# liyangSKD/slam-eslam

Measured on AMD Instinct MI355X. Metric: M particle-updates/s (predict+weight+resample) @ 1/2/4/8 MI355X, higher is better.
Workload: dtype f64; 1 GPU; configs[2]: 4194304 particles/GPU, 1 MI355X per rank, MLS 1000x1000 @0.1 m, 4 contacts, resample forced every step; particles_per_gpu=4194304, global_particles=4194304, parallelism=dp1 (particle shards)

## Files before the change

include/eslam_detmath.h:

```cpp
#ifndef ESLAM_DETMATH_H
#define ESLAM_DETMATH_H

#include <stdint.h>

#if defined(__HIPCC__)
#define DM_FN __host__ __device__ static inline __attribute__((always_inline))
#define DM_CONST static constexpr
#define DM_UNROLL _Pragma("unroll")
#else
#define DM_FN static inline
#define DM_CONST static const
#define DM_UNROLL
#endif

DM_FN uint64_t dm_bits(double x) { uint64_t u; __builtin_memcpy(&u, &x, 8); return u; }
DM_FN double dm_from_bits(uint64_t u) { double x; __builtin_memcpy(&x, &u, 8); return x; }
DM_FN uint32_t dm_fbits(float x) { uint32_t u; __builtin_memcpy(&u, &x, 4); return u; }
DM_FN int dm_isnan(double x) { return x != x; }
DM_FN int dm_isfinite(double x) { return (dm_bits(x) & 0x7ff0000000000000ull) != 0x7ff0000000000000ull; }
DM_FN double dm_fabs(double x) { return dm_from_bits(dm_bits(x) & 0x7fffffffffffffffull); }
DM_FN double dm_fma(double a, double b, double c) { return __builtin_fma(a, b, c); }
#if defined(__HIP_DEVICE_COMPILE__)
DM_FN double dm_fmak(double a, double b, double k)
{
// ... 757 lines not shown
    {-0.47139673682599764, 0.881921264348355},
    {-0.4496113296546066, 0.8932243011955153},
    {-0.4275550934302821, 0.9039892931234433},
    {-0.40524131400498986, 0.9142097557035307},
    {-0.3826834323650898, 0.9238795325112867},
    {-0.35989503653498817, 0.9329927988347388},
    {-0.33688985339222005, 0.9415440651830208},
    {-0.31368174039889146, 0.9495281805930367},
    {-0.2902846772544624, 0.9569403357322088},
    {-0.26671275747489837, 0.9637760657954398},
    {-0.2429801799032639, 0.970031253194544},
    {-0.2191012401568698, 0.9757021300385286},
    {-0.19509032201612828, 0.9807852804032304},
    {-0.17096188876030122, 0.9852776423889412},
    {-0.14673047445536175, 0.989176509964781},
    {-0.1224106751992162, 0.99247953459871},
    {-0.0980171403295606, 0.9951847266721969},
    {-0.07356456359966743, 0.9972904566786902},
    {-0.049067674327418015, 0.9987954562051724},
    {-0.024541228522912288, 0.9996988186962042},
};
#define DM_BM_DELTA 1.4629180792671596e-09

DM_FN double dm_log_bm(double u)
{
    const uint64_t b = dm_bits(u);
    const uint32_t hi = (uint32_t)(b >> 32);
    const int32_t t = (int32_t)(hi - 0x3fe80000u);
    const int32_t k = t >> 20;
    const uint32_t i = ((uint32_t)t >> 13) & 127u;
    const double z = dm_from_bits(((uint64_t)(hi - ((uint32_t)t & 0xfff00000u)) << 32) | (b & 0xffffffffull));
    const double* e = dm_bm_log_tab[i];
    const double r = dm_fma(z, e[0], -1.0);
    double p = dm_fmak(r, 1.0 / 7.0, -1.0 / 6.0);
    p = dm_fmak(p, r, 0.2);
    p = dm_fmak(p, r, -0.25);
    p = dm_fmak(p, r, 1.0 / 3.0);
    p = dm_fma_mh(p, r);
    const double l1p = dm_fma(r * r, p, r);
    const double kd = (double)k;
    const double h = kd * DM_LN2_HI + e[1];
    const double l = kd * DM_LN2_LO + e[2];
    return h + (l1p + l);
}

DM_FN void dm_sincos2pi32(uint32_t b, double* s, double* c)
{
    const double* e = dm_bm_sc_tab[b >> 24];
    const double d = ((double)(b & 0xffffffu) + 0.5) * DM_BM_DELTA;
    const double z = d * d;
    double ps = dm_fmak(z, -1.0 / 5040.0, 1.0 / 120.0);
    ps = dm_fmak(ps, z, -1.0 / 6.0);
    const double sd = dm_fma(d * z, ps, d);
    double pc = dm_fmak(z, 1.0 / 40320.0, -1.0 / 720.0);
    pc = dm_fmak(pc, z, 1.0 / 24.0);
    pc = dm_fma_mh(pc, z);
    const double cd = dm_fma_1(pc, z);
    *s = dm_fma(e[0], cd, e[1] * sd);
    *c = dm_fma(e[1], cd, -(e[0] * sd));
}

DM_CONST float dm_bm_sc_tab32[256][2] = {
    {0.0f, 1.0f},
    {0.024541229009628296f, 0.99969881772995f},
    {0.049067676067352295f, 0.9987954497337341f},
    {0.0735645666718483f, 0.9972904324531555f},
// ... 234 lines not shown
    {-0.4275550842285156f, 0.903989315032959f},
    {-0.40524131059646606f, 0.91420978307724f},
    {-0.3826834261417389f, 0.9238795042037964f},
    {-0.3598950505256653f, 0.9329928159713745f},
    {-0.3368898630142212f, 0.9415440559387207f},
    {-0.3136817514896393f, 0.949528157711029f},
    {-0.290284663438797f, 0.9569403529167175f},
    {-0.2667127549648285f, 0.9637760519981384f},
    {-0.24298018217086792f, 0.9700312614440918f},
    {-0.21910123527050018f, 0.9757021069526672f},
    {-0.19509032368659973f, 0.9807852506637573f},
    {-0.1709618866443634f, 0.9852776527404785f},
    {-0.1467304676771164f, 0.9891765117645264f},
    {-0.12241067737340927f, 0.9924795627593994f},
    {-0.0980171412229538f, 0.9951847195625305f},
    {-0.0735645666718483f, 0.9972904324531555f},
    {-0.049067676067352295f, 0.9987954497337341f},
    {-0.024541229009628296f, 0.99969881772995f},
};
#define DM_BM_DELTA_F 1.462918119976564e-09f

DM_FN float dm_fmaf(float a, float b, float c) { return __builtin_fmaf(a, b, c); }

DM_FN void dm_sincos2pi32f(uint32_t b, float* s, float* c)
{
    const float* e = dm_bm_sc_tab32[b >> 24];
    const float d = dm_fmaf((float)(b & 0xffffffu), DM_BM_DELTA_F, 0.5f * DM_BM_DELTA_F);
    const float z = d * d;
    const float sd = dm_fmaf(d * z, -1.0f / 6.0f, d);
    const float cd = dm_fmaf(z, dm_fmaf(z, 1.0f / 24.0f, -0.5f), 1.0f);
    *s = dm_fmaf(e[0], cd, e[1] * sd);
    *c = dm_fmaf(e[1], cd, -(e[0] * sd));
}

DM_FN float dm_sqrtf_pos(float x)
{
#if defined(__HIP_DEVICE_COMPILE__)
    const float r = __builtin_amdgcn_sqrtf(x);
    const float dn = __uint_as_float(__float_as_uint(r) - 1u), up = __uint_as_float(__float_as_uint(r) + 1u);
    float q = r;
    if (__builtin_fmaf(-dn, r, x) <= 0.0f) q = dn;
    if (__builtin_fmaf(-up, r, x) > 0.0f) q = up;
    return q;
#else
    return __builtin_sqrtf(x);
#endif
}

DM_FN void dm_box_muller32(uint32_t a, uint32_t b, double* z0, double* z1)
{
    const float r = dm_sqrtf_pos((float)(-2.0 * dm_log_bm(dm_u32(a))));
    float s, c;
    dm_sincos2pi32f(b, &s, &c);
    *z0 = (double)r * (double)c;
    *z1 = (double)r * (double)s;
}

#define DM_STREAM_PROJECT 1u
#define DM_STREAM_INIT 2u
#define DM_STREAM_HASH 3u

DM_FN dm_philox_ctr dm_draw(uint64_t seed, uint32_t stream, uint64_t ev, uint64_t gidx, uint32_t call)
{
    dm_philox_ctr c;
    c.v[0] = (uint32_t)gidx;
    c.v[1] = (uint32_t)(gidx >> 32);
    c.v[2] = (uint32_t)ev;
    c.v[3] = (stream << 24) | ((call & 0xffu) << 16) | (uint32_t)((ev >> 32) & 0xffffu);
    return dm_philox4x32_10(c, (uint32_t)seed, (uint32_t)(seed >> 32) ^ 0x5EED5EEDu);
}

#define DM_MINSTD_A 48271u
#define DM_MINSTD_M 2147483647u

DM_FN uint32_t dm_mulmod31(uint32_t a, uint32_t b)
{
    uint64_t p = (uint64_t)a * b;
    uint64_t r = (p & DM_MINSTD_M) + (p >> 31);
// ... 578 lines not shown
```

slam-eslam_amd/csrc/eslam_internal.h:

```cpp
#pragma once
#include <stdint.h>
#include "../../include/eslam_gpu.h"
#include "../../include/eslam_detmath.h"

namespace eslam_dev {

constexpr int kBlock = 256;
constexpr int kWaves = kBlock / 64;
constexpr int kScanItems = 8;
constexpr int kScanTile = kBlock * kScanItems;
constexpr int kGatherTile = kScanTile;
constexpr int kRow = 64;
constexpr int kNShard = 16;
constexpr int kJumpBits = 11;
constexpr int kStatsLds = 2048;
#ifndef ESLAM_WINDOW_LDS
#define ESLAM_WINDOW_LDS 29696
#endif
constexpr int kWindowLds = ESLAM_WINDOW_LDS;
#ifndef ESLAM_K1_ATTR
#define ESLAM_K1_ATTR
#endif

#if defined(__HIPCC__)
__device__ __forceinline__ uint32_t jump_pow(const uint32_t* __restrict__ jt, uint64_t e)
{
    uint32_t a = jt[e & 2047u];
    uint32_t b = jt[2048u + ((e >> 11) & 2047u)];
    uint32_t c = jt[4096u + ((e >> 22) & 1023u)];
    return dm_mulmod31(dm_mulmod31(a, b), c);
}
#endif

struct alignas(128) Shard {
    uint64_t A[DM_NBUCKETS][4];
    uint64_t B[DM_NBUCKETS][4];
    uint64_t SW[4];
    uint64_t D, TP;
    uint64_t maxm;
    uint64_t flags;
    uint64_t err;
    uint64_t bbox[4];
// ... 414 lines not shown
```

slam-eslam_amd/csrc/eslam_kernels.hip:

```cpp
#include <hip/hip_runtime.h>
#include <type_traits>
#include <string.h>

#include "eslam_internal.h"
#include "eslam_launch.h"

namespace eslam_dev {

template <int O> __device__ __forceinline__ uint32_t xor_lane_u32(uint32_t v)
{
    static_assert(O == 1 || O == 2 || O == 4 || O == 8 || O == 16 || O == 32, "xor distance");
    if constexpr (O == 32) {
        const auto r = __builtin_amdgcn_permlane32_swap(v, v, false, false);
        return (threadIdx.x & 32u) ? r[0] : r[1];
    } else if constexpr (O == 16) {
        const auto r = __builtin_amdgcn_permlane16_swap(v, v, false, false);
        return (threadIdx.x & 16u) ? r[0] : r[1];
    } else if constexpr (O == 8) {
        const int t = __builtin_amdgcn_update_dpp(0, (int)v, 0x108, 0xf, 0x3, false);
        return (uint32_t)__builtin_amdgcn_update_dpp(t, (int)v, 0x118, 0xf, 0xc, false);
    } else if constexpr (O == 4) {
        const int t = __builtin_amdgcn_update_dpp(0, (int)v, 0x104, 0xf, 0x5, false);
        return (uint32_t)__builtin_amdgcn_update_dpp(t, (int)v, 0x114, 0xf, 0xa, false);
    } else if constexpr (O == 2) {
// ... 121 lines not shown
{
    su2 r;
    asm volatile("s_load_dwordx2 %0, %1, %2\n\ts_waitcnt lgkmcnt(0)" : "=&s"(r) : "s"(kseg()), "s"(off));
    return r;
}
__device__ __forceinline__ su4 kl4(uint32_t off)
{
    su4 r;
    asm volatile("s_load_dwordx4 %0, %1, %2\n\ts_waitcnt lgkmcnt(0)" : "=&s"(r) : "s"(kseg()), "s"(off));
    return r;
}
__device__ __forceinline__ su8 kl8(uint32_t off)
{
    su8 r;
    asm volatile("s_load_dwordx8 %0, %1, %2\n\ts_waitcnt lgkmcnt(0)" : "=&s"(r) : "s"(kseg()), "s"(off));
    return r;
}
__device__ __forceinline__ su16 kl16(uint32_t off)
{
    su16 r;
    asm volatile("s_load_dwordx16 %0, %1, %2\n\ts_waitcnt lgkmcnt(0)" : "=&s"(r) : "s"(kseg()), "s"(off));
    return r;
}
__device__ __forceinline__ void kl8_2(uint32_t off_a, uint32_t off_b, su8& a, su2& b)
{
    asm volatile("s_load_dwordx8 %0, %2, %3\n\ts_load_dwordx2 %1, %2, %4\n\ts_waitcnt lgkmcnt(0)"
                 : "=&s"(a), "=&s"(b) : "s"(kseg()), "s"(off_a), "s"(off_b));
}
template <class V> __device__ __forceinline__ uint64_t kq(const V& r, int k)
{
    return (uint64_t)r[2 * k] | ((uint64_t)r[2 * k + 1] << 32);
}
template <class V> __device__ __forceinline__ double kd(const V& r, int k) { return dm_from_bits(kq(r, k)); }
template <class T> using gmem = __attribute__((address_space(1))) T;
template <class T, class V> __device__ __forceinline__ gmem<T>* kp(const V& r, int k) { return (gmem<T>*)(uintptr_t)kq(r, k); }

struct StatePtrs {
    gmem<double> *x, *y, *th, *z, *zs, *w, *mprob;
    gmem<uint8_t>* flags;
};
__device__ __forceinline__ StatePtrs kstate(uint32_t off)
{
    const su16 r = kl16(off);
    return StatePtrs{kp<double>(r, 0), kp<double>(r, 1), kp<double>(r, 2), kp<double>(r, 3),
                     kp<double>(r, 4), kp<double>(r, 5), kp<double>(r, 6), kp<uint8_t>(r, 7)};
}

static_assert(offsetof(StepParams, mu) == 24 && offsetof(StepParams, L22) == 88 && offsetof(StepParams, z_delta) == 120 &&
                  offsetof(StepParams, me2) == 136 && offsetof(StepParams, use_shape) == 168,
              "K1 scalar-load blocks");
static_assert(offsetof(MapView, width) == 48 && offsetof(MapView, height) == 64, "map lookup header");
static_assert(offsetof(ContactC, pz) == 32 && offsetof(GatherView, record) == 32, "K1 scalar-load blocks");
static_assert(offsetof(LocalMaps, S) == 24 && offsetof(LocalMaps, hy) == 40 && offsetof(LocalMaps, mx) == 48 &&
                  offsetof(LocalMaps, my) == 56, "K1 reads the local maps' first 64 bytes");

struct alignas(16) WinCell {
    float mean0, stdev0;
    uint32_t begin, count;
};

__shared__ __attribute__((aligned(16))) int k1_win[8];

struct Window {
    int on;
    const WinCell* cells;
};

struct WinBounds {
    int on, m0, m1, n0, n1, cols;
// ... 101 lines not shown
    for (int i = 0; i < N; ++i) {
        if (dm[i] == 0xffffffffu) continue;
        if (pg[i] == kStoreTrail) {
            fnd[i] = store_patch(sid, dm[i], dn[i], lz[i], qv, mean[i], stdev[i]);
        } else if (pg[i] != DM_LM_NONE) {
            const float sd = __uint_as_float((uint32_t)(pf[i] >> 32));
            fnd[i] = dm_lm_holds(sd) && patch_gate(nullptr, 0, __uint_as_float((uint32_t)pf[i]), sd, lz[i], qv, mean[i], stdev[i]);
        }
    }
}

__device__ __forceinline__ uint32_t store_sid(uint32_t sid)
{
    const su16 h = kl16(KOFF(store));
    const uint64_t w3 = kq(h, 3), w5 = kq(h, 5);
    const uint32_t S = (uint32_t)w3, V = (uint32_t)(w5 >> 32);
    const uint32_t f = kp<const uint32_t>(h, 1)[(uint64_t)sid * S + (S - 4u * V - 2u)];
    return sid | (f == kLmShadow ? 0x80000000u : 0u);
}

template <bool DELTA = false, bool DEFER = false>
__device__ __forceinline__ bool get_patch(const Window& win, double px, double py, double pz, double qv, double& mean,
                                          double& stdev, uint32_t sid = 0, uint32_t* dm = nullptr, uint32_t* dn = nullptr,
                                          double* dlz = nullptr)
{
    if constexpr (DEFER) *dm = 0xffffffffu;
    const su16 h = kl16(KOFF(map));
    const uint32_t width = h[12], hcells = h[13], ident = h[14], has_height = h[15];
    double lx = px, ly = py, lz = pz;
    if (!ident) {
        const su16 a = kl16(KOFF(map.g2l));
        const su8 b = kl8(KOFF(map.g2l[8]));
        lx = ((kd(a, 0) * px + kd(a, 1) * py) + kd(a, 2) * pz) + kd(a, 3);
        ly = ((kd(a, 4) * px + kd(a, 5) * py) + kd(a, 6) * pz) + kd(a, 7);
        lz = ((kd(b, 0) * px + kd(b, 1) * py) + kd(b, 2) * pz) + kd(b, 3);
    }
    const double ux = (lx - kd(h, 4)) * kd(h, 2);
    const double uy = (ly - kd(h, 5)) * kd(h, 3);
    if constexpr (DELTA) {
        if (sid >> 31) {
            sid &= 0x7fffffffu;
            const double fm = floor(ux), fn = floor(uy);
            if ((fm >= 0.0) & (fm < (double)width) & (fn >= 0.0) & (fn < (double)hcells) &&
                store_patch(sid, (uint32_t)fm, (uint32_t)fn, lz, qv, mean, stdev))
                return true;
        }
    }
    int im, in;
    asm("v_cvt_i32_f64 %0, %1" : "=v"(im) : "v"(ux));
    asm("v_cvt_i32_f64 %0, %1" : "=v"(in) : "v"(uy));
// ... 151 lines not shown
    return w;
}

struct CMResult {
    uint32_t ncp;
    bool accepted;
    double weight, zdelta, zvar, posevar, s2;
};

__device__ __forceinline__ bool ratio_surely_significant(double z, double zvar, double corr)
{
    const double s2 = zvar * (corr * corr);
    if (z <= 0.0) return s2 < 1e16;
    return s2 < 1600.0 && z * z < 31.36 * s2;
}

#ifndef ESLAM_K1_LB
#define ESLAM_K1_LB 4
#endif
constexpr int kK1LookupBatch = ESLAM_K1_LB;

template <int MAXP, bool BATCH, bool DELTA = false, bool UNG = false>
__device__ __forceinline__ CMResult evaluate_pose(const Window& win, double co, double s, double r22, double x, double y,
                                                  double z, double meas_var, uint32_t sid)
{
    CMResult r;
    double cz[MAXP], cv[MAXP];
    bool ok[MAXP];
#pragma unroll
    for (int k = 0; k < MAXP; ++k) ok[k] = false;
    uint32_t ncp = 0;
    bool valid = false, group_valid = true;
    double contact_ratio = 0, pose_var_avg = 0, posevar = 0;
    double pzd = 0, pzv = 0;
    const double qv = meas_var;
    const su8 wp = kl8(KOFF(p.me2));
    const su4 wq = kl4(KOFF(p.use_shape));
    const double radius = kd(wp, 1), corr = kd(wp, 2);
    const uint32_t m = wq[1], eval_mask = wq[2], end_mask = wq[3];

    auto push = [&](uint32_t i, double zd, double zv) {
        if constexpr (BATCH) {
            cz[i] = zd; cv[i] = zv; ok[i] = true;
        } else {
#pragma unroll
            for (int k = 0; k < MAXP; ++k)
                if ((uint32_t)k == ncp) { cz[k] = zd; cv[k] = zv; }
        }
        ++ncp;
    };
    auto contact = [&](uint32_t i, bool found, double mean, double stdev, double wz) {
        const bool c_eval = (eval_mask >> i) & 1u, c_end = (end_mask >> i) & 1u;
        if (group_valid && c_eval) {
            if (found) {
                const double zdiff = wz - mean;
                const double pose_var = stdev * stdev;
                const double zvar = stdev * stdev + meas_var;
                if (!valid && c_end && ratio_surely_significant(zdiff, zvar, corr)) {
                    posevar += pose_var;
                    push(i, zdiff, zvar);
// ... 14 lines not shown
                    pzv += zvar * ratio;
                    contact_ratio += ratio;
                    pose_var_avg += pose_var * ratio;
                }
                valid = true;
            } else {
                group_valid = false;
            }
        }
        if (valid && c_end) {
            if (group_valid && contact_ratio > 1e-9) {
                const double inv = 1.0 / contact_ratio;
                pzd *= inv;
                pzv *= inv;
                posevar += pose_var_avg * inv;
                push(i, pzd, pzv);
            }
            group_valid = true;
            valid = false;
            pose_var_avg = 0;
            contact_ratio = 0;
        }
    };
    auto world = [&](uint32_t i, double& wx, double& wy, double& wz) {
        su8 c;
        su2 cpz;
        const uint32_t off = KOFF(p.c) + i * (uint32_t)sizeof(ContactC);
        kl8_2(off, off + (uint32_t)offsetof(ContactC, pz), c, cpz);
        const double px = kd(c, 0), py = kd(c, 1), zp = kd(c, 2), zz = kd(c, 3), pz = kd(cpz, 0);
        wx = ((co * px + (-s) * py) + zp) + x;
        wy = ((s * px + co * py) + zp) + y;
        wz = ((zz + r22 * pz) + z) - radius;
    };
    auto lookup = [&](double wx, double wy, double wz, double& mean, double& stdev) -> bool {
        return get_patch<DELTA>(win, wx, wy, wz, qv, mean, stdev, sid);
    };

    if constexpr (BATCH && UNG && kK1LookupBatch < MAXP) {
        bool alive = true;
#pragma unroll
        for (int g = 0; g < MAXP; g += kK1LookupBatch) {
            bool fnd[kK1LookupBatch];
            double mn[kK1LookupBatch], sd[kK1LookupBatch], wzs[kK1LookupBatch];
#pragma unroll
            for (int q = 0; q < kK1LookupBatch; ++q) {
                const int i = g + q;
                fnd[q] = false; mn[q] = 0.0; sd[q] = 0.0; wzs[q] = 0.0;
                if ((uint32_t)i < m) {
                    double wx, wy;
                    world((uint32_t)i, wx, wy, wzs[q]);
                    if ((eval_mask >> i) & 1u) fnd[q] = lookup(wx, wy, wzs[q], mn[q], sd[q]);
                }
            }
#pragma unroll
            for (int q = 0; q < kK1LookupBatch; ++q) {
                const int i = g + q;
                if ((uint32_t)i >= m) break;
                if (!((eval_mask >> i) & 1u)) continue;
                if (alive && fnd[q]) {
                    const double zdiff = wzs[q] - mn[q];
                    const double pose_var = sd[q] * sd[q];
                    const double zvar = sd[q] * sd[q] + meas_var;
                    double pzd_i = zdiff, pzv_i = zvar, pv_i = pose_var;
                    bool take = true;
                    if (!ratio_surely_significant(zdiff, zvar, corr)) {
                        const double ratio = dm_normal_pdf_cdf_ratio(zdiff, dm_sqrt(zvar) * corr);
                        take = ratio > 1e-9;
                        const double inv = 1.0 / ratio;
                        pzd_i = (zdiff * ratio) * inv;
                        pzv_i = (zvar * ratio) * inv;
                        pv_i = (pose_var * ratio) * inv;
                    }
                    if (take) {
                        posevar += pv_i;
                        push((uint32_t)i, pzd_i, pzv_i);
                    }
                }
                alive = alive && fnd[q];
            }
        }
    } else if constexpr (BATCH) {
        bool fnd[MAXP];
        double mn[MAXP], sd[MAXP], wzs[MAXP];
        if constexpr (DELTA) {
            if (!(sid >> 31)) {
                uint32_t dm[MAXP], dn[MAXP];
                double dlz[MAXP];
#pragma unroll
                for (int i = 0; i < MAXP; ++i) {
                    fnd[i] = false; mn[i] = 0.0; sd[i] = 0.0; wzs[i] = 0.0; dm[i] = 0xffffffffu; dn[i] = 0u; dlz[i] = 0.0;
                    if ((uint32_t)i < m) {
                        double wx, wy;
                        world((uint32_t)i, wx, wy, wzs[i]);
                        if ((eval_mask >> i) & 1u)
                            fnd[i] = get_patch<true, true>(win, wx, wy, wzs[i], qv, mn[i], sd[i], sid, &dm[i], &dn[i], &dlz[i]);
                    }
                }
                store_patches<MAXP>(sid, dm, dn, dlz, qv, fnd, mn, sd);
            } else {
#pragma unroll
                for (int i = 0; i < MAXP; ++i) {
                    fnd[i] = false; mn[i] = 0.0; sd[i] = 0.0; wzs[i] = 0.0;
                    if ((uint32_t)i < m) {
                        double wx, wy;
                        world((uint32_t)i, wx, wy, wzs[i]);
                        if ((eval_mask >> i) & 1u) fnd[i] = lookup(wx, wy, wzs[i], mn[i], sd[i]);
                    }
                }
            }
        } else {
#pragma unroll
            for (int i = 0; i < MAXP; ++i) {
                fnd[i] = false; mn[i] = 0.0; sd[i] = 0.0; wzs[i] = 0.0;
                if ((uint32_t)i < m) {
                    double wx, wy;
                    world((uint32_t)i, wx, wy, wzs[i]);
                    if ((eval_mask >> i) & 1u) fnd[i] = lookup(wx, wy, wzs[i], mn[i], sd[i]);
                }
            }
        }
        if constexpr (UNG) {
            bool alive = true;
#pragma unroll
            for (int i = 0; i < MAXP; ++i) {
                if ((uint32_t)i >= m) break;
                if (!((eval_mask >> i) & 1u)) continue;
                if (alive && fnd[i]) {
                    const double zdiff = wzs[i] - mn[i];
                    const double pose_var = sd[i] * sd[i];
                    const double zvar = sd[i] * sd[i] + meas_var;
                    double pzd_i = zdiff, pzv_i = zvar, pv_i = pose_var;
                    bool take = true;
                    if (!ratio_surely_significant(zdiff, zvar, corr)) {
                        const double ratio = dm_normal_pdf_cdf_ratio(zdiff, dm_sqrt(zvar) * corr);
                        take = ratio > 1e-9;
                        const double inv = 1.0 / ratio;
                        pzd_i = (zdiff * ratio) * inv;
                        pzv_i = (zvar * ratio) * inv;
                        pv_i = (pose_var * ratio) * inv;
                    }
                    if (take) {
                        posevar += pv_i;
                        push((uint32_t)i, pzd_i, pzv_i);
                    }
                }
                alive = alive && fnd[i];
            }
        } else {
#pragma unroll
            for (int i = 0; i < MAXP; ++i) {
                if ((uint32_t)i >= m) break;
                contact((uint32_t)i, fnd[i], mn[i], sd[i], wzs[i]);
            }
        }
    } else {
        for (uint32_t i = 0; i < m; ++i) {
            double wx, wy, wz, mean = 0.0, stdev = 0.0;
            world(i, wx, wy, wz);
            bool found = false;
            if (group_valid && ((eval_mask >> i) & 1u)) found = lookup(wx, wy, wz, mean, stdev);
            contact(i, found, mean, stdev, wz);
        }
    }
    r.ncp = ncp;
    r.posevar = posevar;
    r.accepted = (uint64_t)ncp >= kq(wp, 3);
    r.weight = r.zdelta = r.zvar = r.s2 = 0.0;
    if (r.accepted) {
        double d1 = 0, d2 = 0, inv_d2;
        auto sums = [&](auto recip) {
#pragma unroll
            for (int k = 0; k < MAXP; ++k) {
                if (BATCH ? ok[k] : (uint32_t)k < ncp) {
                    cv[k] = recip(cv[k]);
                    d1 += cz[k] * cv[k];
                    d2 += cv[k];
                }
            }
            inv_d2 = recip(d2);
        };
        if (meas_var >= 0x1p-400 && meas_var <= 0x1p300) sums([](double v) { return dm_div_inrange(1.0, v); });
        else sums([](double v) { return 1.0 / v; });
        const double delta = d1 * inv_d2;
        double s2 = 0.0;
#pragma unroll
        for (int k = 0; k < MAXP; ++k) {
            if (BATCH ? ok[k] : (uint32_t)k < ncp) {
                const double d = cz[k] - delta;
                s2 += (d * d) * cv[k];
            }
        }
        r.s2 = s2;
        const uint32_t use_shape = kl2(KOFF(p.use_shape))[0];
        const double pz = use_shape ? dm_exp(-0.5 * s2) : 1.0;
        r.weight = pz;
        r.zdelta = -delta;
        r.zvar = inv_d2;
    }
    return r;
}

__device__ __forceinline__ uint32_t decode_source(uint32_t v, uint32_t multi, const gmem<const Rec>* __restrict__ recs,
                                                  const gmem<const Rec>** rec)
{
    *rec = nullptr;
    if (multi) {
        if (v >= kMarkOwn && v < kMarkHigh) return v - kMarkOwn;
        *rec = recs + (v >= kMarkHigh ? v - kMarkHigh : v);
        return 0;
    }
    return v;
}

#define K1_ST(p, v) __builtin_nontemporal_store((v), (p))

#ifndef ESLAM_K1D_WPE
// ... 10 lines not shown
    const uint64_t nchunks = (n + csz - 1) / csz;
    Ctl* ctl = a.ctl;
    if (ctl->err & kFaultTimeout) return;
    const uint32_t gath = ctl->gather;
    const uint32_t cur = ctl->base ^ ctl->flip;
    if (WEIGHT && blockIdx.x == 0 && threadIdx.x == 0) ctl->k3_base = cur;
    const uint32_t st_off = __builtin_amdgcn_readfirstlane(cur ? KOFF(s[1]) : KOFF(s[0]));
    const uint32_t si_off = __builtin_amdgcn_readfirstlane(gath ? (ctl->base ? KOFF(s[1]) : KOFF(s[0])) : st_off);
    const int wexp = ctl->wexp;
    double spread = 0.0;
    bool do_spread = false;
    double tf = 0.0, rf = 0.0;
    if (PROJECT) {
        spread = dm_weighting_function(ctl->max_weight, 0.0, a.p.spread_threshold, 0.0);
        do_spread = spread > 0 && !a.p.hash_use;
        tf = a.p.spread_trans * spread;
        rf = a.p.spread_rot * spread;
    }

    extern __shared__ __attribute__((aligned(16))) unsigned char smem[];
    Window win;
    win.on = 0;
    if (WEIGHT) win = stage_window(a.map, a.p, ctl, 6.0 * tf, smem + kStatsLds);
    ESLAM_STAMP(g_stamps_k1, 1);

    double maxm = 0.0;
    uint32_t nDTP = 0, werr = 0, flag = 0;
    uint32_t touched = 0;
    float bb[4] = {-INFINITY, -INFINITY, -INFINITY, -INFINITY};
    uint64_t limb = 0;
    const int sa = DM_FX_SCALE - wexp, sb = DM_FX_SCALE - 2 * wexp;

    uint64_t chunk = (uint64_t)blockIdx.x * kWaves + wave;
    bool active = chunk < nchunks;
    if (a.sel.mode == 1u) {
        active = chunk >= a.sel.cdev[0] && chunk < a.sel.cdev[1];
    } else if (a.sel.mode == 2u) {
        chunk = chunk < a.sel.c_lo ? chunk : a.sel.c_hi + (chunk - a.sel.c_lo);
        active = chunk < nchunks;
    }
    if (active) {
    const uint64_t lbase = chunk * csz;
    constexpr uint32_t kNoBucket = 0xffu;
    double curA = 0.0, curB = 0.0;
    uint32_t cur_b = kNoBucket;
    constexpr bool kRegAcc = DELTA;
    double accA[kRegAcc ? DM_NBUCKETS : 1], accB[kRegAcc ? DM_NBUCKETS : 1];
#pragma unroll
    for (int k = 0; k < (kRegAcc ? DM_NBUCKETS : 1); ++k) accA[k] = accB[k] = 0.0;
    double accSW = 0.0;

    for (uint32_t j = 0; j < J; ++j) {
        const uint64_t row0 = lbase + 64ull * j;
        if (row0 >= n) break;
        const uint64_t i = row0 + lane;
        uint32_t src = (uint32_t)i;
        const gmem<const Rec>* rc = nullptr;
        uint32_t rec_anc = 0;
        bool clr = false;
        if (gath) {
            const su8 g = kl8(KOFF(gv));
            const su2 gf = kl2(KOFF(gv.record));
            gmem<uint32_t>* marks = kp<uint32_t>(g, 0);
            const uint32_t carry = kp<const uint32_t>(g, 1)[row0 / kRow] + 1u;
            uint32_t m = 0;
            if (i < n) { m = marks[i]; clr = m != 0; }
            m = wave_incl_max_u32(m);
            m = m > carry ? m : carry;
            src = decode_source(m - 1u, gf[1], kp<const Rec>(g, 3), &rc);
            rec_anc = gf[0];
        }
        uint32_t bucket = kNoBucket;
        double am = 0.0, am2 = 0.0;
        bool rowerr = false;
        if (i < n) {
        double x, y, th, z, zs, w, mp_in = 0.0;
        uint32_t fl_in = 0;
        if (rc) {
            x = rc->x; y = rc->y; th = rc->th; z = rc->z; zs = rc->zs; w = rc->w;
            mp_in = rc->mprob; fl_in = (uint8_t)rc->src;
        } else {
            const StatePtrs si = kstate(si_off);
            x = si.x[src]; y = si.y[src]; th = si.th[src]; z = si.z[src];
            zs = si.zs[src]; w = si.w[src];
            if (!WEIGHT && gath) { mp_in = si.mprob[src]; fl_in = si.flags[src]; }
        }
        if (gath && rec_anc) {
            const su2 ga = kl2(KOFF(gv.anc));
            const uint64_t gbase = kq(kl2(KOFF(p.gbase)), 0);
            kp<uint32_t>(ga, 0)[i] = rc ? (uint32_t)(rc->src >> 8) : (uint32_t)(gbase + src);
        }
        const double w_in = w;
        double mprob = 0.0;
        uint32_t flags = 0;
        if (PROJECT) {
            const su8 key = kl8(KOFF(p.seed));
            const uint64_t gi = kq(key, 2) + i;
            const dm_philox_ctr d0 = dm_draw(kq(key, 0), DM_STREAM_PROJECT, kq(key, 1), gi, 0);
            const dm_philox_ctr d1 = dm_draw(kq(key, 0), DM_STREAM_PROJECT, kq(key, 1), gi, 1);
            double z0, z1, z2, sn0;
            dm_box_muller32(d0.v[0], d0.v[1], &z0, &z1);
            dm_box_muller32(d0.v[2], d0.v[3], &z2, &sn0);
            const su16 P = kl16(KOFF(p.mu));
            const su8 Q = kl8(KOFF(p.L22));
            const double dx = kd(P, 0) + kd(P, 3) * z0;
            double dy = kd(P, 1) + (kd(P, 4) * z0 + kd(P, 5) * z1);
            const double dth = kd(P, 2) + ((kd(P, 6) * z0 + kd(P, 7) * z1) + kd(Q, 0) * z2);
            if (dm_u32(d1.v[0]) < kd(Q, 1)) dy *= dm_u32(d1.v[1]);
            double s, co;
            dm_sincos(th, &s, &co);
            x += co * dx - s * dy;
            y += s * dx + co * dy;
            th += dth;
            if (kd(Q, 3) > 0.0) {
                if (dm_fabs(th - kd(Q, 2)) > kd(Q, 3)) w *= 0.7;
            }
            const su4 Z = kl4(KOFF(p.z_delta));
            z += kd(Z, 0);
            zs = dm_sqrt_fast(zs * zs + kd(Z, 1));
            if (do_spread) {
                double sn1, sn2;
                dm_box_muller32(d1.v[2], d1.v[3], &sn1, &sn2);
                x += sn0 * tf + 0.0;
                y += sn1 * tf + 0.0;
                th += sn2 * rf + 0.0;
            }
        }
        if (WEIGHT) {
            double s, co;
            dm_sincos(th, &s, &co);
            const double r22 = (1.0 - co) + co;
            const double meas_var = zs * zs + kd(kl2(KOFF(p.me2)), 0);
            uint32_t sid = 0;
            if constexpr (DELTA) {
                sid = store_sid(kp<const uint32_t>(kl2(st_off + (uint32_t)offsetof(DevState, sid)), 0)[i]);
            }
            CMResult r = evaluate_pose<MAXP, BATCH, DELTA, UNG>(win, co, s, r22, x, y, z, meas_var, sid);
            if (meas_var == 0) {
                rowerr = true;
                r.accepted = false;
                r.ncp = 0;
            }
            uint32_t floating;
            double sw = 0.0;
            if (r.accepted) {
                double zvar = zs * zs;
                const double inv_n = dm_recip_small(r.ncp);
                double pose_var;
                if (r.ncp != 0u && (r.ncp & (r.ncp - 1u)) == 0u) pose_var = r.posevar * inv_n;
                else pose_var = r.posevar / (double)r.ncp;
                const double av = zvar - pose_var;
                double delta_var = (av < 1e-9) ? 1e-9 : av;
                if (!(r.zdelta * r.zdelta > delta_var)) {
                    const double gain = zvar / (zvar + r.zvar);
                    z += gain * r.zdelta;
                    const double var_gain = delta_var / (delta_var + r.zvar);
                    delta_var = (1.0 - var_gain) * delta_var;
                    zvar = pose_var + delta_var;
                }
                zs = dm_sqrt_fast(zvar);
                if (r.ncp == 0u) {
                    z = dm_from_bits(0x7ff8000000000000ull);
                    zs = dm_from_bits(0x7ff8000000000000ull);
                }
                w *= r.weight;
                mprob = r.weight;
                floating = 0;
                maxm = (maxm < r.weight) ? r.weight : maxm;
                nDTP += 1u + (r.ncp << 16);
                const uint32_t use_shape = kl2(KOFF(p.use_shape))[0];
                if (!use_shape || r.ncp == 0) sw = dm_pow(r.weight, inv_n);
                else sw = r.weight == 0.0 ? 0.0 : dm_exp((-0.5 * r.s2) * inv_n);
            } else {
                floating = 1;
                mprob = 1.0;
            }
            bucket = r.ncp < DM_NBUCKETS - 1 ? r.ncp : DM_NBUCKETS - 1;
            am = w * mprob;
            am2 = am * am;
            accSW = accSW + sw;
            flags = (r.ncp & 0x7fu) | (floating << 7);
        } else {
            mprob = mp_in;
            flags = fl_in;
        }
        const StatePtrs st = kstate(st_off);
        if (PROJECT || gath) {
            K1_ST(st.x + i, x);
            K1_ST(st.y + i, y);
            K1_ST(st.th + i, th);
        }
        if (WEIGHT || gath) {
            K1_ST(st.mprob + i, mprob);
            K1_ST(st.flags + i, (uint8_t)flags);
        }
        if (PROJECT || WEIGHT) {
            K1_ST(st.z + i, z);
            K1_ST(st.zs + i, zs);
            if (gath || w != w_in || w != w) K1_ST(st.w + i, w);
        }
        if (clr) kp<uint32_t>(kl2(KOFF(gv.marks)), 0)[i] = 0;
        {
            const float xf = (float)x, yf = (float)y;
            bb[0] = __builtin_fmaxf(bb[0], -xf);
            bb[1] = __builtin_fmaxf(bb[1], xf);
            bb[2] = __builtin_fmaxf(bb[2], -yf);
            bb[3] = __builtin_fmaxf(bb[3], yf);
        }
        }
        if (WEIGHT) {
            werr |= __ballot(rowerr) != 0ull ? 1u : 0u;
            uint64_t todo = __ballot(bucket != kNoBucket);
            while (todo) {
                const uint32_t b0 = (uint32_t)__builtin_amdgcn_readlane((int)bucket, (int)__builtin_ctzll(todo));
                const bool mine = bucket == b0;
                if constexpr (kRegAcc) {
                    touched |= 1u << b0;
#pragma unroll
                    for (uint32_t k = 0; k < (uint32_t)DM_NBUCKETS; ++k) {
                        if (k == b0) {
                            accA[k] = accA[k] + (mine ? am : 0.0);
                            accB[k] = accB[k] + (mine ? am2 : 0.0);
                        }
                    }
// ... 2641 lines not shown
    for (uint64_t a = (uint64_t)blockIdx.x * kBlock + threadIdx.x; a < (1ull << 32); a += stride) {
        const float x = (float)(-2.0 * dm_log_bm(dm_u32((uint32_t)a)));
        cnt += __float_as_uint(dm_sqrtf_pos(x)) != __float_as_uint(__builtin_sqrtf(x)) ? 1u : 0u;
    }
    cnt = wave_sum_u32(cnt);
    if ((threadIdx.x & 63u) == 0 && cnt) atomicAdd(bad, (unsigned long long)cnt);
}

}

using namespace eslam_dev;

static uint32_t k1_grid(uint64_t chunks) { return (uint32_t)((chunks + kWaves - 1) / kWaves); }

extern "C" hipError_t eslam_launch_project_weight(int project, int weight, int maxp, DevState s0, DevState s1,
                                                  const MapView* map, const StepParams* p, Ctl* ctl, Shard* shards,
                                                  const GatherView* gv, const LocalMaps* store, hipStream_t stream,
                                                  const ChunkSel* sel, double* bspill)
{
    const uint64_t csz = 64ull * p->J;
    uint64_t chunks = (p->n + csz - 1) / csz;
    if (sel && sel->mode == 2u) chunks = sel->c_lo + (chunks > sel->c_hi ? chunks - sel->c_hi : 0);
    if (chunks == 0) return hipSuccess;
    const size_t lds = kStatsLds + (weight ? kWindowLds : 0);
    K1Args args;
    args.p = *p;
    args.map = *map;
    args.gv = *gv;
    args.s[0] = s0;
    args.s[1] = s1;
    args.ctl = ctl;
    args.shards = shards;
    memset(&args.store, 0, sizeof(args.store));
    if (store) args.store = *store;
    memset(&args.sel, 0, sizeof(args.sel));
    if (sel) args.sel = *sel;
    args.bspill = bspill;
    if (weight && !bspill) return hipErrorInvalidValue;
#define ESLAM_LAUNCH(P, W, M, B, ...)                                                                   \
    hipLaunchKernelGGL((k_project_weight<P, W, M, B, ##__VA_ARGS__>), dim3(k1_grid(chunks)), dim3(kBlock), lds, \
                       stream, args)
    const uint32_t all = p->m >= 32 ? 0xffffffffu : ((1u << p->m) - 1u);
    const bool ung = (p->end_mask & all) == all;
    if (weight && store) {
        if (p->m <= 4 && maxp <= 4) {
            if (project) { if (ung) ESLAM_LAUNCH(true, true, 4, true, true, true); else ESLAM_LAUNCH(true, true, 4, true, true); }
            else { if (ung) ESLAM_LAUNCH(false, true, 4, true, true, true); else ESLAM_LAUNCH(false, true, 4, true, true); }
// ... 616 lines not shown
```

Baseline: 16830 M particle-updates/s.

## Stage Box-Muller tables in LDS and batch scalar parameter loads

Box-Muller log and sincos lookup tables are copied into LDS per block, placed in the tail of the window region when the window leaves room, and the table rows are fetched early, right after the Philox draws. Draws are also hoisted ahead of the gather decode so the math overlaps with the marks load. Several separate scalar constant loads (map header, contact data, weight params, state pointers, marks pointer) are merged into grouped s_load sequences with a single wait, which removes repeated lgkmcnt stalls. The cost is extra LDS use and a block barrier in project-only launches, plus scheduling barriers that constrain the compiler.

```diff
diff --git a/include/eslam_detmath.h b/include/eslam_detmath.h
--- a/include/eslam_detmath.h
+++ b/include/eslam_detmath.h
@@ -803,15 +803,20 @@
 };
 #define DM_BM_DELTA 1.4629180792671596e-09
 
-DM_FN double dm_log_bm(double u)
+DM_FN uint32_t dm_log_bm_row(double u)
+{
+    const int32_t t = (int32_t)((uint32_t)(dm_bits(u) >> 32) - 0x3fe80000u);
+    return ((uint32_t)t >> 13) & 127u;
+}
+
+DM_FN double dm_log_bm_e(double u, double e0, double e1, double e2)
 {
     const uint64_t b = dm_bits(u);
     const uint32_t hi = (uint32_t)(b >> 32);
     const int32_t t = (int32_t)(hi - 0x3fe80000u);
     const int32_t k = t >> 20;
-    const uint32_t i = ((uint32_t)t >> 13) & 127u;
     const double z = dm_from_bits(((uint64_t)(hi - ((uint32_t)t & 0xfff00000u)) << 32) | (b & 0xffffffffull));
-    const double* e = dm_bm_log_tab[i];
+    const double e[3] = {e0, e1, e2};
     const double r = dm_fma(z, e[0], -1.0);
     double p = dm_fmak(r, 1.0 / 7.0, -1.0 / 6.0);
     p = dm_fmak(p, r, 0.2);
@@ -823,6 +828,12 @@
     const double h = kd * DM_LN2_HI + e[1];
     const double l = kd * DM_LN2_LO + e[2];
     return h + (l1p + l);
+}
+
+DM_FN double dm_log_bm(double u)
+{
+    const double* e = dm_bm_log_tab[dm_log_bm_row(u)];
+    return dm_log_bm_e(u, e[0], e[1], e[2]);
 }
 
 DM_FN void dm_sincos2pi32(uint32_t b, double* s, double* c)
@@ -1103,15 +1114,20 @@
 
 DM_FN float dm_fmaf(float a, float b, float c) { return __builtin_fmaf(a, b, c); }
 
-DM_FN void dm_sincos2pi32f(uint32_t b, float* s, float* c)
-{
-    const float* e = dm_bm_sc_tab32[b >> 24];
+DM_FN void dm_sincos2pi32f_e(uint32_t b, float e0, float e1, float* s, float* c)
+{
     const float d = dm_fmaf((float)(b & 0xffffffu), DM_BM_DELTA_F, 0.5f * DM_BM_DELTA_F);
     const float z = d * d;
     const float sd = dm_fmaf(d * z, -1.0f / 6.0f, d);
     const float cd = dm_fmaf(z, dm_fmaf(z, 1.0f / 24.0f, -0.5f), 1.0f);
-    *s = dm_fmaf(e[0], cd, e[1] * sd);
-    *c = dm_fmaf(e[1], cd, -(e[0] * sd));
+    *s = dm_fmaf(e0, cd, e1 * sd);
+    *c = dm_fmaf(e1, cd, -(e0 * sd));
+}
+
+DM_FN void dm_sincos2pi32f(uint32_t b, float* s, float* c)
+{
+    const float* e = dm_bm_sc_tab32[b >> 24];
+    dm_sincos2pi32f_e(b, e[0], e[1], s, c);
 }
 
 DM_FN float dm_sqrtf_pos(float x)
@@ -1128,13 +1144,33 @@
 #endif
 }
 
-DM_FN void dm_box_muller32(uint32_t a, uint32_t b, double* z0, double* z1)
-{
-    const float r = dm_sqrtf_pos((float)(-2.0 * dm_log_bm(dm_u32(a))));
+typedef struct {
+    double l0, l1, l2;
     float s, c;
-    dm_sincos2pi32f(b, &s, &c);
+} dm_bm_rows_t;
+
+DM_FN dm_bm_rows_t dm_bm_rows(uint32_t a, uint32_t b)
+{
+    const double* l = dm_bm_log_tab[dm_log_bm_row(dm_u32(a))];
+    const float* e = dm_bm_sc_tab32[b >> 24];
+    dm_bm_rows_t t;
+    t.l0 = l[0]; t.l1 = l[1]; t.l2 = l[2];
+    t.s = e[0]; t.c = e[1];
+    return t;
+}
+
+DM_FN void dm_box_muller32_e(uint32_t a, uint32_t b, dm_bm_rows_t t, double* z0, double* z1)
+{
+    const float r = dm_sqrtf_pos((float)(-2.0 * dm_log_bm_e(dm_u32(a), t.l0, t.l1, t.l2)));
+    float s, c;
+    dm_sincos2pi32f_e(b, t.s, t.c, &s, &c);
     *z0 = (double)r * (double)c;
     *z1 = (double)r * (double)s;
+}
+
+DM_FN void dm_box_muller32(uint32_t a, uint32_t b, double* z0, double* z1)
+{
+    dm_box_muller32_e(a, b, dm_bm_rows(a, b), z0, z1);
 }
 
 #define DM_STREAM_PROJECT 1u
diff --git a/slam-eslam_amd/csrc/eslam_internal.h b/slam-eslam_amd/csrc/eslam_internal.h
--- a/slam-eslam_amd/csrc/eslam_internal.h
+++ b/slam-eslam_amd/csrc/eslam_internal.h
@@ -18,6 +18,11 @@
 #define ESLAM_WINDOW_LDS 29696
 #endif
 constexpr int kWindowLds = ESLAM_WINDOW_LDS;
+#ifndef ESLAM_K1_BM_LDS
+#define ESLAM_K1_BM_LDS 1
+#endif
+constexpr int kBmLds = 6144;
+static_assert(kBmLds <= kWindowLds, "the tables lie inside the window's LDS");
 #ifndef ESLAM_K1_ATTR
 #define ESLAM_K1_ATTR
 #endif
diff --git a/slam-eslam_amd/csrc/eslam_kernels.hip b/slam-eslam_amd/csrc/eslam_kernels.hip
--- a/slam-eslam_amd/csrc/eslam_kernels.hip
+++ b/slam-eslam_amd/csrc/eslam_kernels.hip
@@ -167,11 +167,25 @@
     asm volatile("s_load_dwordx16 %0, %1, %2\n\ts_waitcnt lgkmcnt(0)" : "=&s"(r) : "s"(kseg()), "s"(off));
     return r;
 }
-__device__ __forceinline__ void kl8_2(uint32_t off_a, uint32_t off_b, su8& a, su2& b)
-{
-    asm volatile("s_load_dwordx8 %0, %2, %3\n\ts_load_dwordx2 %1, %2, %4\n\ts_waitcnt lgkmcnt(0)"
-                 : "=&s"(a), "=&s"(b) : "s"(kseg()), "s"(off_a), "s"(off_b));
-}
+#define ESLAM_KL_GROUP2(name, WA, WB) \
+    __device__ __forceinline__ void name(su##WA& a, uint32_t off_a, su##WB& b, uint32_t off_b) \
+    { \
+        asm volatile("s_load_dwordx" #WA " %0, %2, %3\n\ts_load_dwordx" #WB " %1, %2, %4\n\ts_waitcnt lgkmcnt(0)" \
+                     : "=&s"(a), "=&s"(b) : "s"(kseg()), "s"(off_a), "s"(off_b)); \
+    }
+#define ESLAM_KL_GROUP3(name, WA, WB, WC) \
+    __device__ __forceinline__ void name(su##WA& a, uint32_t off_a, su##WB& b, uint32_t off_b, su##WC& c, uint32_t off_c) \
+    { \
+        asm volatile("s_load_dwordx" #WA " %0, %3, %4\n\ts_load_dwordx" #WB " %1, %3, %5\n\ts_load_dwordx" #WC \
+                     " %2, %3, %6\n\ts_waitcnt lgkmcnt(0)" \
+                     : "=&s"(a), "=&s"(b), "=&s"(c) : "s"(kseg()), "s"(off_a), "s"(off_b), "s"(off_c)); \
+    }
+ESLAM_KL_GROUP2(kl8_2, 8, 2)
+ESLAM_KL_GROUP2(kl8_4, 8, 4)
+ESLAM_KL_GROUP2(kl16_2, 16, 2)
+ESLAM_KL_GROUP3(kl8_2_8, 8, 2, 8)
+ESLAM_KL_GROUP3(kl8_2_16, 8, 2, 16)
+ESLAM_KL_GROUP3(kl16_8_4, 16, 8, 4)
 template <class V> __device__ __forceinline__ uint64_t kq(const V& r, int k)
 {
     return (uint64_t)r[2 * k] | ((uint64_t)r[2 * k + 1] << 32);
@@ -184,12 +198,12 @@
     gmem<double> *x, *y, *th, *z, *zs, *w, *mprob;
     gmem<uint8_t>* flags;
 };
-__device__ __forceinline__ StatePtrs kstate(uint32_t off)
-{
-    const su16 r = kl16(off);
+__device__ __forceinline__ StatePtrs state_ptrs(const su16& r)
+{
     return StatePtrs{kp<double>(r, 0), kp<double>(r, 1), kp<double>(r, 2), kp<double>(r, 3),
                      kp<double>(r, 4), kp<double>(r, 5), kp<double>(r, 6), kp<uint8_t>(r, 7)};
 }
+__device__ __forceinline__ StatePtrs kstate(uint32_t off) { return state_ptrs(kl16(off)); }
 
 static_assert(offsetof(StepParams, mu) == 24 && offsetof(StepParams, L22) == 88 && offsetof(StepParams, z_delta) == 120 &&
                   offsetof(StepParams, me2) == 136 && offsetof(StepParams, use_shape) == 168,
@@ -337,10 +351,10 @@
 template <bool DELTA = false, bool DEFER = false>
 __device__ __forceinline__ bool get_patch(const Window& win, double px, double py, double pz, double qv, double& mean,
                                           double& stdev, uint32_t sid = 0, uint32_t* dm = nullptr, uint32_t* dn = nullptr,
-                                          double* dlz = nullptr)
+                                          double* dlz = nullptr, const su16* hin = nullptr)
 {
     if constexpr (DEFER) *dm = 0xffffffffu;
-    const su16 h = kl16(KOFF(map));
+    const su16 h = hin ? *hin : kl16(KOFF(map));
     const uint32_t width = h[12], hcells = h[13], ident = h[14], has_height = h[15];
     double lx = px, ly = py, lz = pz;
     if (!ident) {
@@ -538,7 +552,7 @@
 
 template <int MAXP, bool BATCH, bool DELTA = false, bool UNG = false>
 __device__ __forceinline__ CMResult evaluate_pose(const Window& win, double co, double s, double r22, double x, double y,
-                                                  double z, double meas_var, uint32_t sid)
+                                                  double z, double meas_var, uint32_t sid, const su8& wp, const su4& wq)
 {
     CMResult r;
     double cz[MAXP], cv[MAXP];
@@ -550,8 +564,6 @@
     double contact_ratio = 0, pose_var_avg = 0, posevar = 0;
     double pzd = 0, pzv = 0;
     const double qv = meas_var;
-    const su8 wp = kl8(KOFF(p.me2));
-    const su4 wq = kl4(KOFF(p.use_shape));
     const double radius = kd(wp, 1), corr = kd(wp, 2);
     const uint32_t m = wq[1], eval_mask = wq[2], end_mask = wq[3];
 
@@ -612,18 +624,18 @@
             contact_ratio = 0;
         }
     };
-    auto world = [&](uint32_t i, double& wx, double& wy, double& wz) {
+    auto world = [&](uint32_t i, double& wx, double& wy, double& wz, su16& h) {
         su8 c;
         su2 cpz;
         const uint32_t off = KOFF(p.c) + i * (uint32_t)sizeof(ContactC);
-        kl8_2(off, off + (uint32_t)offsetof(ContactC, pz), c, cpz);
+        kl8_2_16(c, off, cpz, off + (uint32_t)offsetof(ContactC, pz), h, KOFF(map));
         const double px = kd(c, 0), py = kd(c, 1), zp = kd(c, 2), zz = kd(c, 3), pz = kd(cpz, 0);
         wx = ((co * px + (-s) * py) + zp) + x;
         wy = ((s * px + co * py) + zp) + y;
         wz = ((zz + r22 * pz) + z) - radius;
     };
-    auto lookup = [&](double wx, double wy, double wz, double& mean, double& stdev) -> bool {
-        return get_patch<DELTA>(win, wx, wy, wz, qv, mean, stdev, sid);
+    auto lookup = [&](const su16& h, double wx, double wy, double wz, double& mean, double& stdev) -> bool {
+        return get_patch<DELTA>(win, wx, wy, wz, qv, mean, stdev, sid, nullptr, nullptr, nullptr, &h);
     };
 
     if constexpr (BATCH && UNG && kK1LookupBatch < MAXP) {
@@ -638,8 +650,9 @@
                 fnd[q] = false; mn[q] = 0.0; sd[q] = 0.0; wzs[q] = 0.0;
                 if ((uint32_t)i < m) {
                     double wx, wy;
-                    world((uint32_t)i, wx, wy, wzs[q]);
-                    if ((eval_mask >> i) & 1u) fnd[q] = lookup(wx, wy, wzs[q], mn[q], sd[q]);
+                    su16 h;
+                    world((uint32_t)i, wx, wy, wzs[q], h);
+                    if ((eval_mask >> i) & 1u) fnd[q] = lookup(h, wx, wy, wzs[q], mn[q], sd[q]);
                 }
             }
 #pragma unroll
@@ -681,9 +694,10 @@
                     fnd[i] = false; mn[i] = 0.0; sd[i] = 0.0; wzs[i] = 0.0; dm[i] = 0xffffffffu; dn[i] = 0u; dlz[i] = 0.0;
                     if ((uint32_t)i < m) {
                         double wx, wy;
-                        world((uint32_t)i, wx, wy, wzs[i]);
+                        su16 h;
+                        world((uint32_t)i, wx, wy, wzs[i], h);
                         if ((eval_mask >> i) & 1u)
-                            fnd[i] = get_patch<true, true>(win, wx, wy, wzs[i], qv, mn[i], sd[i], sid, &dm[i], &dn[i], &dlz[i]);
+                            fnd[i] = get_patch<true, true>(win, wx, wy, wzs[i], qv, mn[i], sd[i], sid, &dm[i], &dn[i], &dlz[i], &h);
                     }
                 }
                 store_patches<MAXP>(sid, dm, dn, dlz, qv, fnd, mn, sd);
@@ -693,8 +707,9 @@
                     fnd[i] = false; mn[i] = 0.0; sd[i] = 0.0; wzs[i] = 0.0;
                     if ((uint32_t)i < m) {
                         double wx, wy;
-                        world((uint32_t)i, wx, wy, wzs[i]);
-                        if ((eval_mask >> i) & 1u) fnd[i] = lookup(wx, wy, wzs[i], mn[i], sd[i]);
+                        su16 h;
+                        world((uint32_t)i, wx, wy, wzs[i], h);
+                        if ((eval_mask >> i) & 1u) fnd[i] = lookup(h, wx, wy, wzs[i], mn[i], sd[i]);
                     }
                 }
             }
@@ -704,8 +719,9 @@
                 fnd[i] = false; mn[i] = 0.0; sd[i] = 0.0; wzs[i] = 0.0;
                 if ((uint32_t)i < m) {
                     double wx, wy;
-                    world((uint32_t)i, wx, wy, wzs[i]);
-                    if ((eval_mask >> i) & 1u) fnd[i] = lookup(wx, wy, wzs[i], mn[i], sd[i]);
+                    su16 h;
+                    world((uint32_t)i, wx, wy, wzs[i], h);
+                    if ((eval_mask >> i) & 1u) fnd[i] = lookup(h, wx, wy, wzs[i], mn[i], sd[i]);
                 }
             }
         }
@@ -746,9 +762,10 @@
     } else {
         for (uint32_t i = 0; i < m; ++i) {
             double wx, wy, wz, mean = 0.0, stdev = 0.0;
-            world(i, wx, wy, wz);
+            su16 h;
+            world(i, wx, wy, wz, h);
             bool found = false;
-            if (group_valid && ((eval_mask >> i) & 1u)) found = lookup(wx, wy, wz, mean, stdev);
+            if (group_valid && ((eval_mask >> i) & 1u)) found = lookup(h, wx, wy, wz, mean, stdev);
             contact(i, found, mean, stdev, wz);
         }
     }
@@ -781,7 +798,7 @@
             }
         }
         r.s2 = s2;
-        const uint32_t use_shape = kl2(KOFF(p.use_shape))[0];
+        const uint32_t use_shape = wq[0];
         const double pz = use_shape ? dm_exp(-0.5 * s2) : 1.0;
         r.weight = pz;
         r.zdelta = -delta;
@@ -838,6 +855,22 @@
     Window win;
     win.on = 0;
     if (WEIGHT) win = stage_window(a.map, a.p, ctl, 6.0 * tf, smem + kStatsLds);
+    unsigned char* bm_tab = smem + kStatsLds + (WEIGHT ? kWindowLds - kBmLds : 0);
+    uint32_t bm_lds = 0;
+    if (ESLAM_K1_BM_LDS && PROJECT) {
+        static_assert(sizeof(dm_bm_log_tab) == 4096 && sizeof(dm_bm_sc_tab32) == 2048 && kBlock == 256, "one piece per thread");
+        int room = 1;
+        if (win.on) {
+            const WinBounds wb = win_bounds();
+            room = (wb.n1 - wb.n0) * wb.cols * (int)sizeof(WinCell) <= kWindowLds - kBmLds;
+        }
+        bm_lds = (uint32_t)__builtin_amdgcn_readfirstlane(room);
+        if (bm_lds) {
+            reinterpret_cast<uint4*>(bm_tab)[threadIdx.x] = reinterpret_cast<const uint4*>(&dm_bm_log_tab[0][0])[threadIdx.x];
+            reinterpret_cast<uint2*>(bm_tab + 4096)[threadIdx.x] = reinterpret_cast<const uint2*>(&dm_bm_sc_tab32[0][0])[threadIdx.x];
+        }
+        __syncthreads();
+    }
     ESLAM_STAMP(g_stamps_k1, 1);
 
     double maxm = 0.0;
@@ -874,17 +907,52 @@
         const gmem<const Rec>* rc = nullptr;
         uint32_t rec_anc = 0;
         bool clr = false;
+        dm_philox_ctr d0 = {}, d1 = {};
+        dm_bm_rows_t t0 = {}, t1 = {};
+        su8 key = {};
+        auto draws = [&]() {
+            if (!PROJECT) return;
+            const uint64_t gi = kq(key, 2) + i;
+            d0 = dm_draw(kq(key, 0), DM_STREAM_PROJECT, kq(key, 1), gi, 0);
+            d1 = dm_draw(kq(key, 0), DM_STREAM_PROJECT, kq(key, 1), gi, 1);
+            asm volatile("" ::"v"(d0.v[0]), "v"(d0.v[1]), "v"(d0.v[2]), "v"(d0.v[3]), "v"(d1.v[0]), "v"(d1.v[1]),
+                         "v"(d1.v[2]), "v"(d1.v[3]));
+        };
         if (gath) {
-            const su8 g = kl8(KOFF(gv));
-            const su2 gf = kl2(KOFF(gv.record));
-            gmem<uint32_t>* marks = kp<uint32_t>(g, 0);
+            su8 g;
+            su2 gf;
+            if constexpr (PROJECT) kl8_2_8(g, KOFF(gv), gf, KOFF(gv.record), key, KOFF(p.seed));
+            else kl8_2(g, KOFF(gv), gf, KOFF(gv.record));
             const uint32_t carry = kp<const uint32_t>(g, 1)[row0 / kRow] + 1u;
-            uint32_t m = 0;
-            if (i < n) { m = marks[i]; clr = m != 0; }
+            uint32_t m = kp<uint32_t>(g, 0)[i < n ? i : n - 1];
+            draws();
+            m = i < n ? m : 0u;
+            clr = m != 0;
             m = wave_incl_max_u32(m);
             m = m > carry ? m : carry;
             src = decode_source(m - 1u, gf[1], kp<const Rec>(g, 3), &rc);
             rec_anc = gf[0];
+        } else {
+            if constexpr (PROJECT) key = kl8(KOFF(p.seed));
+            draws();
+        }
+        if (PROJECT) {
+            if (bm_lds) {
+                auto rows = [&](uint32_t wa, uint32_t wb) {
+                    const double* l = reinterpret_cast<const double*>(bm_tab) + 4 * dm_log_bm_row(dm_u32(wa));
+                    const float* e = reinterpret_cast<const float*>(bm_tab + 4096) + 2 * (wb >> 24);
+                    dm_bm_rows_t t;
+                    t.l0 = l[0]; t.l1 = l[1]; t.l2 = l[2];
+                    t.s = e[0]; t.c = e[1];
+                    return t;
+                };
+                t0 = rows(d0.v[0], d0.v[1]);
+                t1 = rows(d0.v[2], d0.v[3]);
+            } else {
+                t0 = dm_bm_rows(d0.v[0], d0.v[1]);
+                t1 = dm_bm_rows(d0.v[2], d0.v[3]);
+            }
+            __builtin_amdgcn_sched_barrier(0);
         }
         uint32_t bucket = kNoBucket;
         double am = 0.0, am2 = 0.0;
@@ -910,19 +978,19 @@
         double mprob = 0.0;
         uint32_t flags = 0;
         if (PROJECT) {
-            const su8 key = kl8(KOFF(p.seed));
-            const uint64_t gi = kq(key, 2) + i;
-            const dm_philox_ctr d0 = dm_draw(kq(key, 0), DM_STREAM_PROJECT, kq(key, 1), gi, 0);
-            const dm_philox_ctr d1 = dm_draw(kq(key, 0), DM_STREAM_PROJECT, kq(key, 1), gi, 1);
+            su16 P;
+            su8 Q;
+            su4 Z;
+            kl16_8_4(P, KOFF(p.mu), Q, KOFF(p.L22), Z, KOFF(p.z_delta));
             double z0, z1, z2, sn0;
-            dm_box_muller32(d0.v[0], d0.v[1], &z0, &z1);
-            dm_box_muller32(d0.v[2], d0.v[3], &z2, &sn0);
-            const su16 P = kl16(KOFF(p.mu));
-            const su8 Q = kl8(KOFF(p.L22));
+            dm_box_muller32_e(d0.v[0], d0.v[1], t0, &z0, &z1);
+            dm_box_muller32_e(d0.v[2], d0.v[3], t1, &z2, &sn0);
             const double dx = kd(P, 0) + kd(P, 3) * z0;
             double dy = kd(P, 1) + (kd(P, 4) * z0 + kd(P, 5) * z1);
             const double dth = kd(P, 2) + ((kd(P, 6) * z0 + kd(P, 7) * z1) + kd(Q, 0) * z2);
             if (dm_u32(d1.v[0]) < kd(Q, 1)) dy *= dm_u32(d1.v[1]);
+            asm volatile("" ::"v"(dx), "v"(dy), "v"(dth));
+            __builtin_amdgcn_sched_barrier(0);
             double s, co;
             dm_sincos(th, &s, &co);
             x += co * dx - s * dy;
@@ -931,7 +999,6 @@
             if (kd(Q, 3) > 0.0) {
                 if (dm_fabs(th - kd(Q, 2)) > kd(Q, 3)) w *= 0.7;
             }
-            const su4 Z = kl4(KOFF(p.z_delta));
             z += kd(Z, 0);
             zs = dm_sqrt_fast(zs * zs + kd(Z, 1));
             if (do_spread) {
@@ -946,12 +1013,15 @@
             double s, co;
             dm_sincos(th, &s, &co);
             const double r22 = (1.0 - co) + co;
-            const double meas_var = zs * zs + kd(kl2(KOFF(p.me2)), 0);
+            su8 wp;
+            su4 wq;
+            kl8_4(wp, KOFF(p.me2), wq, KOFF(p.use_shape));
+            const double meas_var = zs * zs + kd(wp, 0);
             uint32_t sid = 0;
             if constexpr (DELTA) {
                 sid = store_sid(kp<const uint32_t>(kl2(st_off + (uint32_t)offsetof(DevState, sid)), 0)[i]);
             }
-            CMResult r = evaluate_pose<MAXP, BATCH, DELTA, UNG>(win, co, s, r22, x, y, z, meas_var, sid);
+            CMResult r = evaluate_pose<MAXP, BATCH, DELTA, UNG>(win, co, s, r22, x, y, z, meas_var, sid, wp, wq);
             if (meas_var == 0) {
                 rowerr = true;
                 r.accepted = false;
@@ -984,7 +1054,7 @@
                 floating = 0;
                 maxm = (maxm < r.weight) ? r.weight : maxm;
                 nDTP += 1u + (r.ncp << 16);
-                const uint32_t use_shape = kl2(KOFF(p.use_shape))[0];
+                const uint32_t use_shape = wq[0];
                 if (!use_shape || r.ncp == 0) sw = dm_pow(r.weight, inv_n);
                 else sw = r.weight == 0.0 ? 0.0 : dm_exp((-0.5 * r.s2) * inv_n);
             } else {
@@ -1000,7 +1070,11 @@
             mprob = mp_in;
             flags = fl_in;
         }
-        const StatePtrs st = kstate(st_off);
+        su16 so;
+        su2 mp = {};
+        if (gath) kl16_2(so, st_off, mp, KOFF(gv.marks));
+        else so = kl16(st_off);
+        const StatePtrs st = state_ptrs(so);
         if (PROJECT || gath) {
             K1_ST(st.x + i, x);
             K1_ST(st.y + i, y);
@@ -1015,7 +1089,7 @@
             K1_ST(st.zs + i, zs);
             if (gath || w != w_in || w != w) K1_ST(st.w + i, w);
         }
-        if (clr) kp<uint32_t>(kl2(KOFF(gv.marks)), 0)[i] = 0;
+        if (clr) kp<uint32_t>(mp, 0)[i] = 0;
         {
             const float xf = (float)x, yf = (float)y;
             bb[0] = __builtin_fmaxf(bb[0], -xf);
@@ -3703,7 +3777,7 @@
     uint64_t chunks = (p->n + csz - 1) / csz;
     if (sel && sel->mode == 2u) chunks = sel->c_lo + (chunks > sel->c_hi ? chunks - sel->c_hi : 0);
     if (chunks == 0) return hipSuccess;
-    const size_t lds = kStatsLds + (weight ? kWindowLds : 0);
+    const size_t lds = kStatsLds + (weight ? kWindowLds : (project && ESLAM_K1_BM_LDS ? kBmLds : 0));
     K1Args args;
     args.p = *p;
     args.map = *map;
```

After: 17770 M particle-updates/s (median of 6 runs). 5.5% higher.
